# matinraayai/ir2rgb

Hardware: AMD Instinct MI355X
Metric: generator+discriminator frames/sec at 512x1024 (higher is better)
Workload: dtype bf16; 1 GPU; vid2vid training window 512x1024: 2-scale generator (composite ngf128 @256x512 + composite-local ngf64 @512x1024, tG=3) + FlowNet2 reference flow + image D (num_D=2) + 2 temporal D, 3 backward passes + Adam; batch 1 frame per GPU; parallelism=dp1 (frame-parallel sequences, RCCL gradient all-reduce)

## Files before the change

ir2rgb_amd/csrc/conv1x7_thin.hip:

```cpp
#include <utility>

#include "common.h"
#include "conv1x7_thin.h"

template <int DT, int CIN>
__global__ void __launch_bounds__(256, 1)
conv1x7_thin_kernel(const uint16_t *__restrict__ X, const uint16_t *__restrict__ Wp, float *__restrict__ Y, const T7Geom g) {
    typedef Half<DT> Hf;
    typedef typename Hf::frag frag;
    constexpr int TW = 128, KW = 7, PAD = 3, ROWS = TW + KW - 1;
    constexpr int NC = CIN / 32;
    constexpr int RB = CIN * 2;
    constexpr int RPI = 1024 / RB;
    constexpr int NDMA = (ROWS + RPI - 1) / RPI;
    constexpr int NDW = (NDMA + 3) / 4;
    constexpr int SEG = NDMA * 1024;
    __shared__ __attribute__((aligned(1024))) unsigned char smem[2 * SEG];

    const int tid = threadIdx.x, lane = tid & 63;
    const int wave = __builtin_amdgcn_readfirstlane(tid >> 6);
    const int l15 = lane & 15, grp = lane >> 4;
    const rsrc_t rx = make_rsrc(X, g.x_bytes);
    const rsrc_t rw = make_rsrc(Wp, g.w_bytes);

    frag A[KW * NC][2];
#pragma unroll
    for (int j = 0; j < KW * NC; ++j) {
        const int kx = j / NC, c = j % NC;
#pragma unroll
        for (int mt = 0; mt < 2; ++mt) {
            const int row = mt * 16 + l15;
            const unsigned off = (unsigned)((((row * (CIN / 64) + (c >> 1)) * KW + kx) * 64 + (c & 1) * 32 + grp * 8) * 2);
            typedef __attribute__((ext_vector_type(4))) unsigned u32x4;
            const u32x4 v = __builtin_amdgcn_raw_buffer_load_b128(rw, row < g.Cout ? off : IR2RGB_OOB, 0, 0);
            A[j][mt] = __builtin_bit_cast(frag, v);
        }
    }

    auto seg_coords = [&](long seg, int &n, int &y, int &x0) {
        const int sx = (int)(seg % g.nsx);
        const long r = seg / g.nsx;
        y = (int)(r % g.H);
        n = (int)(r / g.H);
        x0 = sx * TW;
    };
    auto issue = [&](long seg, int buf) {
        int n, y, x0;
        seg_coords(seg, n, y, x0);
        const unsigned rowbase = (unsigned)(((long)n * g.H + y) * g.W);
#pragma unroll
        for (int q = 0; q < NDW; ++q) {
            const int i = wave + 4 * q;
            const int row = i * RPI + (CIN == 128 ? (lane >> 4) : (lane >> 3));
            const int pos = CIN == 128 ? (lane & 15) : (lane & 7);
            const int chunk = CIN == 128 ? (pos ^ (row & 15)) : (pos ^ ((row >> 1) & 7));
            int xs = x0 - PAD + row;
            xs = xs < 0 ? -xs : xs;
            xs = xs >= g.W ? 2 * g.W - 2 - xs : xs;
            const bool ok = row < ROWS && xs >= 0 && xs < g.W && seg < g.nseg;
            const unsigned v = ok ? ((rowbase + (unsigned)xs) * (unsigned)g.ldx + (unsigned)g.ci_off + (unsigned)chunk * 8u) * 2u : IR2RGB_OOB;
            if (4 * q + 3 < NDMA || i < NDMA)
                lds_dma16(rx, v, 0, smem + buf * SEG + i * 1024);
        }
    };

    const unsigned lds0 = (unsigned)(uintptr_t)(__attribute__((address_space(3))) const unsigned char *)smem;
    unsigned base[KW];
#pragma unroll
    for (int kx = 0; kx < KW; ++kx) {
        const int row = wave * 32 + l15 + kx;
        const int f = CIN == 128 ? (row & 15) : ((row >> 1) & 7);
        base[kx] = lds0 + (unsigned)(row * RB + ((grp ^ f) & (CIN == 128 ? 15 : 7)) * 16);
    }
    constexpr int R = 8, NT = KW * NC * 2;
    auto rd = [&]<int IMM>(frag &dst, unsigned addr, std::integral_constant<int, IMM>) {
        asm volatile("ds_read_b128 %0, %1 offset:%2" : "=v"(dst) : "v"(addr), "n"(IMM) : "memory");
    };

    long seg = blockIdx.x;
    int buf = 0;
    issue(seg, 0);
    for (; seg < g.nseg; seg += gridDim.x) {
        asm volatile("s_waitcnt vmcnt(0) lgkmcnt(0)" ::: "memory");
        __builtin_amdgcn_s_barrier();
        issue(seg + gridDim.x, buf ^ 1);
        const unsigned boff = (unsigned)(buf * SEG);
        f32x4 acc[2][2];
#pragma unroll
        for (int b = 0; b < 2; ++b)
#pragma unroll
            for (int mt = 0; mt < 2; ++mt) acc[b][mt] = (f32x4){0.f, 0.f, 0.f, 0.f};
        frag B[R];
        auto fetch = [&]<int T>(std::integral_constant<int, T>) {
            constexpr int j = T / 2, bb = T % 2, kx = j / NC, c = j % NC;
            rd(B[T % R], (base[kx] ^ (unsigned)(c << 6)) + boff, std::integral_constant<int, bb * 16 * RB>{});
        };
        [&]<int... Ts>(std::integer_sequence<int, Ts...>) { (fetch(std::integral_constant<int, Ts>{}), ...); }(std::make_integer_sequence<int, R>{});
        auto body = [&]<int T>(std::integral_constant<int, T>) {
            constexpr int j = T / 2, bb = T % 2;
            constexpr int after = (NT - 1 - T) < (R - 1) ? (NT - 1 - T) : (R - 1);
            asm volatile("s_waitcnt lgkmcnt(%1)" : "+v"(B[T % R]) : "n"(after) : "memory");
            __builtin_amdgcn_sched_barrier(0);
            acc[bb][0] = Hf::mfma(A[j][0], B[T % R], acc[bb][0]);
            acc[bb][1] = Hf::mfma(A[j][1], B[T % R], acc[bb][1]);
            __builtin_amdgcn_sched_barrier(0);
            if constexpr (T + R < NT) fetch(std::integral_constant<int, T + R>{});
        };
        [&]<int... Ts>(std::integer_sequence<int, Ts...>) { (body(std::integral_constant<int, Ts>{}), ...); }(std::make_integer_sequence<int, NT>{});
        int n, y, x0;
        seg_coords(seg, n, y, x0);
#pragma unroll
        for (int b = 0; b < 2; ++b) {
            const int x = x0 + wave * 32 + b * 16 + l15;
            if (x < g.W) {
                float *dst = Y + (((long)n * g.H + y) * g.W + x) * g.ldy + g.co_off;
#pragma unroll
                for (int mt = 0; mt < 2; ++mt) {
                    const int r0 = mt * 16 + grp * 4;
                    if (r0 + 3 < g.Cout) {
                        *reinterpret_cast<float4 *>(dst + r0) = make_float4(acc[b][mt][0], acc[b][mt][1], acc[b][mt][2], acc[b][mt][3]);
                    } else {
#pragma unroll
                        for (int r = 0; r < 4; ++r)
                            if (r0 + r < g.Cout) dst[r0 + r] = acc[b][mt][r];
                    }
                }
            }
        }
        buf ^= 1;
    }
    asm volatile("s_waitcnt vmcnt(0)" ::: "memory");
}

bool conv1x7_thin_plan(const ir2rgb_conv_desc *d, const ConvView &v, T7Geom *g) {
    if (d->transposed || d->kh != 1 || d->kw != 7 || d->stride_h != 1 || d->stride_w != 1) return false;
    if (d->pad_h != 0 || d->pad_w != 3 || d->pad_mode != 1 || !d->out_f32 || d->act != 0 || d->stats_per_sample) return false;
    if (d->Cout < 1 || d->Cout > 32 || (d->Cin != 64 && d->Cin != 128) || d->Win < 4 || d->Hout != d->Hin || d->Wout != d->Win) return false;
    if (!v.half || (v.ldx & 7) || (d->ci_off & 7) || (v.ldy & 3) || (d->co_off & 3) || v.x_bytes >= (1L << 31)) return false;
    *g = T7Geom{};
    g->N = d->N; g->H = d->Hin; g->W = d->Win; g->Cout = d->Cout;
    g->ldx = v.ldx; g->ci_off = d->ci_off; g->ldy = v.ldy; g->co_off = d->co_off;
    g->nsx = (d->Win + 127) / 128;
    g->nseg = (long)d->N * d->Hin * g->nsx;
    g->x_bytes = (unsigned)v.x_bytes; g->w_bytes = (unsigned)((long)d->Cout * d->Cin * 7 * 2);
    return true;
}

int conv1x7_thin_launch(const T7Geom &g, int dtype, int cin, const void *x, const void *wp, void *y, hipStream_t s) {
    const long want = g.nseg < 512 ? g.nseg : 512;
    const unsigned grid = (unsigned)(want < 1 ? 1 : want);
    with_dtype(dtype, [&](auto dt) {
        auto launch = [&](auto kernel) { kernel<<<grid, 256, 0, s>>>((const uint16_t *)x, (const uint16_t *)wp, (float *)y, g); };
        if (cin == 128) launch(conv1x7_thin_kernel<dt.value, 128>);
        else launch(conv1x7_thin_kernel<dt.value, 64>);
    });
    return ir2rgb_launch_status();
}
```

ir2rgb_amd/csrc/conv_mfma.hip:

```cpp
#include <cstring>
#include <type_traits>
#include <utility>

#include "common.h"
#include "conv1x7_thin.h"
#include "conv3x3_patch.h"
#include "conv7x1_col.h"

#define IR2RGB_MAX_TAPS 49

struct ConvGeom {
    int N, Hin, Win, Cin;
    int Hsub, Wsub;
    int Hout, Wout, Cout;
    int s_in_y, s_in_x;
    int s_out_y, s_out_x, off_y, off_x;
    int ntaps, pad_mode;
    int kchunks;
    int act;
    int ldx, ci_off, ldy, co_off;
    int stats_row0;
    int out_f32;
    FastDiv div_hw, div_w;
    unsigned x_bytes, w_bytes;
    int cout_major;
    int ntx, dy0, dys, dx0, dxs;
    int tpi;
};


template <int TP> struct ConvTile {
    static constexpr int TC = 128;
    static constexpr int STAGE = (TC + TP) * 128;
    static constexpr int NSTAGE = TP == 128 ? 2 : 3;
    static constexpr int LDS = NSTAGE * STAGE;
};

template <int DT, int TP, int NTY, int NTX, int MROWS = 128>
__device__ __forceinline__ void
conv_igemm_body(const uint16_t *__restrict__ X, const uint16_t *__restrict__ Wp, const float *__restrict__ bias,
                uint16_t *__restrict__ Y, float *__restrict__ stats_partial, const ConvGeom &g, const int block,
                unsigned char *const smem) {
    constexpr int TC = 128;
    static_assert(MROWS == 128 || MROWS == 64 || MROWS == 32, "tile rows");
    constexpr int CW = MROWS == 64 ? 32 : 64;
    constexpr int MI = MROWS == 128 ? 4 : 2;
    constexpr int NI = TP / 64;
    constexpr int OC = MROWS <= 64 ? 64 : TC;
    constexpr int WROWS = OC / 64;
    constexpr int PROWS = TP / 64;
    constexpr int LOADS = WROWS + PROWS;
    constexpr int STAGE = (TC + TP) * 128;
    constexpr int NSTAGE = TP == 128 ? 2 : 3;
    constexpr int AHEAD = NSTAGE - 1;
    constexpr bool STATIC_TAPS = NTY > 0;
    constexpr int NT = STATIC_TAPS ? NTY * NTX : 1;
    typedef Half<DT> H;
    typedef typename H::frag frag;

    static_assert(NSTAGE * STAGE == ConvTile<TP>::LDS, "LDS ring size");

    const int tid = threadIdx.x, lane = tid & 63;
    const int wave = __builtin_amdgcn_readfirstlane(tid >> 6);
    const unsigned P = (unsigned)g.N * g.Hsub * g.Wsub;
    const unsigned HW = (unsigned)g.Hsub * g.Wsub;
    const int npt = g.tpi ? g.N * g.tpi : (int)((P + TP - 1) / TP), nct = (g.Cout + TC - 1) / TC;

    int tile;
    {
        const int nwg = npt * nct, b = block, xcd = b & 7, q = nwg >> 3, r = nwg & 7;
        if (b >= nwg) return;
        tile = (xcd < r ? xcd * (q + 1) : r * (q + 1) + (xcd - r) * q) + (b >> 3);
    }
    int pt, ct;
    if (g.cout_major) { ct = tile / npt; pt = tile - ct * npt; }
    else              { pt = tile / nct; ct = tile - pt * nct; }
    unsigned p0 = (unsigned)pt * TP, plim = P, pimg = 0;
    if (g.tpi) { pimg = (unsigned)(pt / g.tpi); p0 = (unsigned)(pt - (int)pimg * g.tpi) * TP; plim = HW; }
    auto pix_decode = [&](unsigned p, unsigned &n, unsigned &rem) {
        if (g.tpi) { n = pimg; rem = p; }
        else { n = fdiv(p, g.div_hw); rem = p - n * HW; }
    };

    const int r8 = tid >> 3, slot = tid & 7;
    const int chunk = slot ^ ((r8 >> 1) & 7);
    const long Ktot = (long)g.kchunks * g.ntaps * 64;

    const rsrc_t rw = make_rsrc(Wp, g.w_bytes), rx = make_rsrc(X, g.x_bytes);
    unsigned woff[WROWS];
#pragma unroll
    for (int i = 0; i < WROWS; ++i) {
        int co = ct * TC + r8 + 64 * i;
        co = co < g.Cout ? co : g.Cout - 1;
        woff[i] = (unsigned)(((long)co * Ktot + chunk * 8) * 2);
    }
    int psy[PROWS], psx[PROWS];
    unsigned pbase[PROWS];
#pragma unroll
    for (int i = 0; i < PROWS; ++i) {
        unsigned p = p0 + r8 + 64 * i;
        const bool v = p < plim;
        p = v ? p : 0u;
        unsigned n, rem;
        pix_decode(p, n, rem);
        unsigned sy = fdiv(rem, g.div_w);
        psy[i] = v ? (int)sy * g.s_in_y : (g.pad_mode ? 0 : -(1 << 20));
        psx[i] = (int)(rem - sy * g.Wsub) * g.s_in_x;
        pbase[i] = n * (unsigned)(g.Hin * g.Win);
    }
    unsigned char *const wave_dst = smem + wave * 1024;

    auto gather_off = [&](int i, int dy, int dx) -> unsigned {
        int iy = psy[i] + dy, ix = psx[i] + dx;
        const bool inb = ((unsigned)iy < (unsigned)g.Hin) & ((unsigned)ix < (unsigned)g.Win);
        iy = g.pad_mode ? reflect(iy, g.Hin) : iy;
        ix = g.pad_mode ? reflect(ix, g.Win) : ix;
        const unsigned off = ((pbase[i] + (unsigned)(iy * g.Win + ix)) * (unsigned)g.ldx + g.ci_off + chunk * 8) * 2u;
        return (g.pad_mode || inb) ? off : IR2RGB_OOB;
    };

    unsigned poff[STATIC_TAPS ? PROWS : 1][NT];
    if constexpr (STATIC_TAPS) {
#pragma unroll
        for (int i = 0; i < PROWS; ++i) {
            int ry[NTY > 0 ? NTY : 1], rx[NTX > 0 ? NTX : 1];
#pragma unroll
            for (int ty = 0; ty < NTY; ++ty) {
                int iy = psy[i] + g.dy0 + ty * g.dys;
                const bool in = (unsigned)iy < (unsigned)g.Hin;
                iy = g.pad_mode ? reflect(iy, g.Hin) : iy;
                ry[ty] = (g.pad_mode || in) ? iy * g.Win : -1;
            }
#pragma unroll
            for (int tx = 0; tx < NTX; ++tx) {
                int ix = psx[i] + g.dx0 + tx * g.dxs;
                const bool in = (unsigned)ix < (unsigned)g.Win;
                ix = g.pad_mode ? reflect(ix, g.Win) : ix;
                rx[tx] = (g.pad_mode || in) ? ix : -1;
            }
            const unsigned cbytes = (unsigned)(g.ci_off + chunk * 8) * 2u, ld2 = (unsigned)g.ldx * 2u;
#pragma unroll
            for (int ty = 0; ty < NTY; ++ty)
#pragma unroll
                for (int tx = 0; tx < NTX; ++tx)
                    poff[i][ty * NTX + tx] = ((ry[ty] | rx[tx]) < 0) ? IR2RGB_OOB
                                                                      : (pbase[i] + (unsigned)(ry[ty] + rx[tx])) * ld2 + cbytes;
        }
    }

    int i_cc = 0, i_ty = 0, i_tx = 0, i_t = 0;
    auto issue_weights = [&](int ks, unsigned char *dst) {
#pragma unroll
        for (int i = 0; i < WROWS; ++i) lds_dma16(rw, woff[i], (unsigned)ks * 128u, dst + 8192 * i);
    };
    auto issue_dynamic = [&](int ks, int buf) {
        unsigned char *dst = wave_dst + buf * STAGE;
        issue_weights(ks, dst);
// ... 407 lines not shown
    int Cout, Cin, T, kind;
    int bx, by;
    int entry, pad_;
};
static inline size_t pack_blocks_offset(int nentries) { return ((size_t)nentries * sizeof(PackEntry) + 15) & ~(size_t)15; }

template <int DT>
__global__ void __launch_bounds__(256)
pack_batch_kernel(const PackEntry *__restrict__ E, const PackBlock *__restrict__ B) {
    __shared__ uint16_t tile[PACK_TILE_HALFS];
    const PackBlock b = B[blockIdx.x];
    if (b.kind == 0) {
        const PackEntry &e = E[b.entry];
        pack_weight_body<DT>(b.w, b.wp, e.g, e.total, b.bx * 256L + threadIdx.x, b.by * 256L);
    } else if (b.kind == 1) {
        pack_tile_body<DT, 0>(b.w, b.wp, b.Cout, b.Cin, b.T, b.bx, b.by, tile);
    } else {
        pack_tile_body<DT, 1>(b.w, b.wp, b.Cout, b.Cin, b.T, b.bx, b.by, tile);
    }
}

struct ClassPlan {
    ConvGeom geom;
    PackGeom pack;
    long w_offset;
    int npt;
    int tp;
};

static int tile_pixels(long P, int Cout, int ksteps) {
    const long nct = (Cout + 127) / 128;
    const long tiles256 = ((P + 255) / 256) * nct;
    if (tiles256 >= 256 && ksteps >= 40) return 256;
    if (((P + 127) / 128) * nct >= 256) return 128;
    return 64;
}

static int make_plan(const ir2rgb_conv_desc *d, const ConvView &v, ClassPlan plans[4]) {
    if (!d || d->N < 1 || d->Cin < 64 || (d->Cin % 64) || d->Cout < 1 || d->kh < 1 || d->kw < 1 ||
        d->kh * d->kw > IR2RGB_MAX_TAPS || d->stride_h < 1 || d->stride_w < 1 || d->pad_h < 0 || d->pad_w < 0)
        return IR2RGB_EINVAL;
    if (!v.half) return IR2RGB_ENOSUP;
    if (d->pad_mode != 0 && d->pad_mode != 1) return IR2RGB_ENOSUP;
    int ncls = 0;
    long woff = 0;
    int row0 = 0;
    auto new_class = [&](int Hsub, int Wsub) -> ClassPlan & {
        ClassPlan &c = plans[ncls++];
        ConvGeom &g = c.geom;
        g = ConvGeom{};
        g.N = d->N; g.Hin = d->Hin; g.Win = d->Win; g.Cin = d->Cin;
        g.Hsub = Hsub; g.Wsub = Wsub; g.Hout = d->Hout; g.Wout = d->Wout; g.Cout = d->Cout;
        g.pad_mode = d->pad_mode; g.kchunks = d->Cin / 64; g.act = d->act; g.out_f32 = d->out_f32;
        c.pack = PackGeom{};
        c.pack.Cout = d->Cout; c.pack.Cin = d->Cin; c.pack.kh = d->kh; c.pack.kw = d->kw; c.pack.transposed = d->transposed ? 1 : 0;
        c.w_offset = woff;
        return c;
    };
    if (!d->transposed) {
        int Ho = (d->Hin + 2 * d->pad_h - d->kh) / d->stride_h + 1, Wo = (d->Win + 2 * d->pad_w - d->kw) / d->stride_w + 1;
        if (Ho != d->Hout || Wo != d->Wout || Ho < 1 || Wo < 1) return IR2RGB_EINVAL;
        if (d->pad_mode == 1 && (d->pad_h >= d->Hin || d->pad_w >= d->Win)) return IR2RGB_EINVAL;
        ClassPlan &c = new_class(Ho, Wo);
        ConvGeom &g = c.geom;
        g.s_in_y = d->stride_h; g.s_in_x = d->stride_w; g.s_out_y = g.s_out_x = 1; g.off_y = g.off_x = 0;
        g.ntaps = c.pack.ntaps = d->kh * d->kw;
        g.ntx = d->kw; g.dy0 = -d->pad_h; g.dys = 1; g.dx0 = -d->pad_w; g.dxs = 1;
        for (int ky = 0, t = 0; ky < d->kh; ++ky)
            for (int kx = 0; kx < d->kw; ++kx, ++t) {
                c.pack.ky[t] = (signed char)ky; c.pack.kx[t] = (signed char)kx;
            }
    } else {
        const int sh = d->stride_h, sw = d->stride_w;
        if (sh > 2 || sw > 2 || d->pad_mode != 0) return IR2RGB_ENOSUP;
        int Hfull = (d->Hin - 1) * sh - 2 * d->pad_h + d->kh, Wfull = (d->Win - 1) * sw - 2 * d->pad_w + d->kw;
        if (d->Hout < Hfull || d->Hout > Hfull + sh - 1 || d->Wout < Wfull || d->Wout > Wfull + sw - 1 || d->Hout < 1 ||
            d->Wout < 1)
            return IR2RGB_EINVAL;
        for (int a = 0; a < sh; ++a)
            for (int b = 0; b < sw; ++b) {
                const int Hsub = (d->Hout - a + sh - 1) / sh, Wsub = (d->Wout - b + sw - 1) / sw;
                if (Hsub < 1 || Wsub < 1) continue;
                ClassPlan &c = new_class(Hsub, Wsub);
                ConvGeom &g = c.geom;
                g.s_in_y = g.s_in_x = 1; g.s_out_y = sh; g.s_out_x = sw; g.off_y = a; g.off_x = b;
                int t = 0, ntx = 0;
                const int ky0 = (a + d->pad_h) % sh, kx0 = (b + d->pad_w) % sw;
                for (int ky = ky0; ky < d->kh; ky += sh) {
                    ntx = 0;
                    for (int kx = kx0; kx < d->kw; kx += sw, ++t, ++ntx) {
                        c.pack.ky[t] = (signed char)ky; c.pack.kx[t] = (signed char)kx;
                    }
                }
                if (t == 0) return IR2RGB_ENOSUP;
                g.ntx = ntx; g.dy0 = (a + d->pad_h - ky0) / sh; g.dys = -1; g.dx0 = (b + d->pad_w - kx0) / sw; g.dxs = -1;
                g.ntaps = c.pack.ntaps = t;
                woff += (long)d->Cout * d->Cin * t;
            }
    }
    if ((long)d->N * d->Hin * d->Win >= (1L << 31) || (long)d->N * d->Hout * d->Wout >= (1L << 31) ||
        (long)d->N * d->Hin * d->Win * (v.ldx / 8) >= 0xFFFFFFFFL)
        return IR2RGB_EINVAL;
    for (int i = 0; i < ncls; ++i) {
        ConvGeom &g = plans[i].geom;
        g.div_hw = make_fastdiv((unsigned)(g.Hsub * g.Wsub)); g.div_w = make_fastdiv((unsigned)g.Wsub);
        g.ldx = v.ldx; g.ci_off = d->ci_off;
        g.ldy = v.ldy; g.co_off = d->co_off;
        if (g.ci_off < 0 || g.co_off < 0 || g.ci_off + d->Cin > g.ldx || g.co_off + d->Cout > g.ldy || (g.ldx & 7) || (g.ci_off & 7))
            return IR2RGB_EINVAL;
        if ((d->Cout & 3) == 0 && ((g.ldy & 3) || (g.co_off & 3))) return IR2RGB_EINVAL;
        const long wb = (long)g.Cout * g.Cin * g.ntaps * 2;
        if (v.x_bytes >= (1L << 31) || wb >= (1L << 31)) return IR2RGB_EINVAL;
        g.x_bytes = (unsigned)v.x_bytes; g.w_bytes = (unsigned)wb;
        g.cout_major = wb > (long)g.N * g.Hin * g.Win * g.Cin * 2 ? 1 : 0;
    }
    int tp_all = 0;
    if (ncls > 1) {
        long p_all = 0, ks_sum = 0;
        for (int i = 0; i < ncls; ++i) {
            const ConvGeom &g = plans[i].geom;
            p_all += (long)g.N * g.Hsub * g.Wsub;
            ks_sum += (long)g.kchunks * g.ntaps;
        }
        tp_all = tile_pixels(p_all, plans[0].geom.Cout, (int)(ks_sum / ncls));
        const long wg128 = ((p_all + 127) / 128) * ((plans[0].geom.Cout + 127) / 128);
        if (tp_all == 128 && wg128 <= 320) tp_all = 64;
    }
    for (int i = 0; i < ncls; ++i) {
        ConvGeom &g = plans[i].geom;
        long P = (long)g.N * g.Hsub * g.Wsub;
        int tp = tp_all ? tp_all : tile_pixels(P, g.Cout, g.kchunks * g.ntaps);
        plans[i].tp = tp;
        plans[i].npt = (int)((P + tp - 1) / tp);
        if (d->stats_per_sample) {
            if (ncls > 1) return IR2RGB_ENOSUP;
            g.tpi = (int)(((long)g.Hsub * g.Wsub + tp - 1) / tp);
            plans[i].npt = g.N * g.tpi;
        }
        g.stats_row0 = row0;
        row0 += plans[i].npt;
    }
    return ncls;
}

extern "C" long ir2rgb_conv2d_packed_weight_elems(const ir2rgb_conv_desc *d) {
    ClassPlan plans[4];
    int n = make_plan(d, conv_view(d), plans);
    if (n < 0) return n;
    long e = 0;
    for (int i = 0; i < n; ++i) e += (long)d->Cout * d->Cin * plans[i].geom.ntaps;
    return e;
}

enum ConvKernel { CONV_IGEMM, CONV_CLASSES, CONV_DOT, CONV_PATCH, CONV_THIN7, CONV_COL7 };
static const char *const CONV_KERNEL_NAMES[] = {"conv_igemm_kernel", "conv_igemm_classes_kernel", "conv_dot_kernel",
                                                "conv3x3_patch_kernel", "conv1x7_thin_kernel", "conv7x1_col_kernel"};
struct ConvRoute {
    ConvKernel kernel;
    int variant;
    P3Geom p3;
    T7Geom t7;
    C7Geom c7;
    int ncls;
    ClassPlan cls[4];
    int stats_rows;
    long workspace_bytes;
};

static bool conv_dot_ok(const ir2rgb_conv_desc *d) {
    static const int v = env_switch("IR2RGB_CONV_DOT", 1);
    return v != 0 && d->out_f32 && d->Cout == 1 && !d->transposed && d->pad_mode == 0 && d->Cin >= 512 && (d->Cin % 512) == 0 &&
           d->kh * d->kw <= 16 && (d->ldx % 8) == 0 && (d->ci_off % 8) == 0;
}

static int conv_route(const ir2rgb_conv_desc *d, bool has_bias, bool has_stats, bool has_workspace, ConvRoute *r) {
    if (!d) return IR2RGB_EINVAL;
    const ConvView v = conv_view(d);
    r->stats_rows = 0; r->workspace_bytes = 0; r->ncls = 0;
    if ((r->variant = conv3x3p_plan(d, v, &r->p3, &r->stats_rows, has_workspace)) != 0) {
        r->kernel = CONV_PATCH;
        r->workspace_bytes = conv3x3p_workspace_bytes(r->variant, r->p3);
        return IR2RGB_OK;
    }
    if (conv7x1_col_plan(d, v, &r->c7)) {
        r->kernel = CONV_COL7;
        r->stats_rows = conv7x1_col_tiles(r->c7);
        return IR2RGB_OK;
    }
    if (!has_bias && !has_stats && conv1x7_thin_plan(d, v, &r->t7)) {
        r->kernel = CONV_THIN7;
        return IR2RGB_OK;
    }
    r->ncls = make_plan(d, v, r->cls);
    if (r->ncls < 0) return r->ncls;
    for (int i = 0; i < r->ncls; ++i) r->stats_rows += r->cls[i].npt;
    r->kernel = r->ncls > 1 ? CONV_CLASSES : !has_stats && conv_dot_ok(d) ? CONV_DOT : CONV_IGEMM;
    return IR2RGB_OK;
}

extern "C" const char *ir2rgb_conv2d_kernel_name(const ir2rgb_conv_desc *d) {
    ConvRoute r;
    return conv_route(d, false, false, false, &r) < 0 ? "" : CONV_KERNEL_NAMES[r.kernel];
}

extern "C" int ir2rgb_conv2d_stats_rows(const ir2rgb_conv_desc *d) {
    ConvRoute r;
    const int rc = conv_route(d, false, true, false, &r);
    return rc < 0 ? rc : r.stats_rows;
}

extern "C" long ir2rgb_conv2d_fwd_workspace_bytes(const ir2rgb_conv_desc *d) {
    ConvRoute r;
    return !d ? IR2RGB_EINVAL : conv_route(d, false, false, true, &r) < 0 ? 0 : r.workspace_bytes;
}

struct PackPlan {
    bool tiled;
    int srcCout, srcCin, T, gx, gy;
    int n;
    PackGeom g[4];
    long w_offset[4], total[4];
};

static int pack_plan(const ir2rgb_conv_desc *d, const void *w, const void *wpacked, bool adjoint, PackPlan *p) {
    ClassPlan plans[4];
    const int n = make_plan(d, conv_view(d), plans);
    if (n < 0) return n;
    if (adjoint && d->transposed) return IR2RGB_ENOSUP;
    const PackGeom &pg = plans[0].pack;
    p->T = d->kh * d->kw;
    bool natural = n == 1 && !d->transposed && pg.ntaps == p->T && p->T <= PACK_MAX_T;
    for (int t = 0; natural && t < p->T; ++t) natural = pg.ky[t] == t / d->kw && pg.kx[t] == t % d->kw;
    p->srcCout = adjoint ? d->Cin : d->Cout; p->srcCin = adjoint ? d->Cout : d->Cin;
    p->tiled = natural && p->srcCin % 64 == 0 && (!adjoint || p->srcCout % 64 == 0) && (((uintptr_t)w | (uintptr_t)wpacked) & 15) == 0;
    const int tco = adjoint ? 64 : 16, tci = adjoint ? 16 : 64;
    p->gx = p->srcCin / tci; p->gy = (p->srcCout + tco - 1) / tco;
    p->n = n;
    for (int i = 0; i < n; ++i) {
        p->g[i] = plans[i].pack;
        if (adjoint) { p->g[i].transposed = 1; p->g[i].flip = 1; }
        p->w_offset[i] = plans[i].w_offset;
        p->total[i] = (long)d->Cout * d->Cin * plans[i].geom.ntaps;
    }
    return IR2RGB_OK;
}

static int pack_impl(const ir2rgb_conv_desc *d, const float *w, void *wpacked, void *stream, bool adjoint) {
    PackPlan p;
    const int rc = pack_plan(d, w, wpacked, adjoint, &p);
    if (rc < 0) return rc;
    uint16_t *dst = reinterpret_cast<uint16_t *>(wpacked);
    hipStream_t s = as_stream(stream);
    with_dtype(d->dtype, [&](auto dt) {
        if (p.tiled) {
            auto tile = [&](auto kernel) { kernel<<<dim3((unsigned)p.gx, (unsigned)p.gy), 256, 0, s>>>(w, dst, p.srcCout, p.srcCin, p.T); };
            if (adjoint) tile(pack_tile_kernel<dt.value, 1>);
            else tile(pack_tile_kernel<dt.value, 0>);
        } else {
            for (int i = 0; i < p.n; ++i)
                pack_weight_kernel<dt.value><<<stream_grid(p.total[i], 256), 256, 0, s>>>(w, dst + p.w_offset[i], p.g[i], p.total[i]);
        }
    });
    return ir2rgb_launch_status();
}

extern "C" int ir2rgb_conv2d_pack_weight(const ir2rgb_conv_desc *d, const float *w, void *wpacked, void *stream) {
    return pack_impl(d, w, wpacked, stream, false);
}

extern "C" int ir2rgb_conv2d_pack_weight_adjoint(const ir2rgb_conv_desc *d, const float *w, void *wpacked, void *stream) {
    return pack_impl(d, w, wpacked, stream, true);
}

static int pack_entries(const ir2rgb_conv_desc *d, const float *w, void *wpacked, bool adjoint, PackEntry *out) {
    PackPlan p;
    const int rc = pack_plan(d, w, wpacked, adjoint, &p);
    if (rc < 0) return rc;
    if (!w || !wpacked) return IR2RGB_EINVAL;
    const int n = p.tiled ? 1 : p.n;
    for (int i = 0; i < n; ++i) {
        PackEntry &e = out[i];
        memset(&e, 0, sizeof(e));
        e.w = w;
        if (p.tiled) {
            e.wp = reinterpret_cast<uint16_t *>(wpacked);
            e.kind = adjoint ? 2 : 1;
            e.Cout = p.srcCout; e.Cin = p.srcCin; e.T = p.T;
            e.gx = p.gx;
            e.nblocks = p.gx * p.gy;
        } else {
            e.g = p.g[i];
            e.total = p.total[i];
            e.wp = reinterpret_cast<uint16_t *>(wpacked) + p.w_offset[i];
            const long nb = (e.total + 1023) / 1024;
            e.nblocks = (int)(nb < 1 ? 1 : (nb > 2048 ? 2048 : nb));
        }
    }
    return n;
}

static int pack_batch_expand(const ir2rgb_pack_job *jobs, int njobs, PackEntry *E, int max_entries, long *nblocks) {
    if (!jobs || njobs < 1) return IR2RGB_EINVAL;
    int n = 0;
    long blocks = 0;
    for (int j = 0; j < njobs; ++j) {
        if (jobs[j].desc.dtype != jobs[0].desc.dtype) return IR2RGB_EINVAL;
        PackEntry tmp[4];
        const int k = pack_entries(&jobs[j].desc, (const float *)jobs[j].w, jobs[j].wpacked, jobs[j].adjoint != 0, tmp);
        if (k < 0) return k;
        for (int i = 0; i < k; ++i) {
            tmp[i].first_block = (int)blocks;
            blocks += tmp[i].nblocks;
            if (E) {
                if (n >= max_entries) return IR2RGB_EINVAL;
                E[n] = tmp[i];
            }
            ++n;
        }
    }
    if (blocks > 0x7fffffffL) return IR2RGB_EINVAL;
    *nblocks = blocks;
    return n;
}

extern "C" long ir2rgb_conv2d_pack_batch_table_bytes(const ir2rgb_pack_job *jobs, int njobs) {
    long blocks = 0;
    const int n = pack_batch_expand(jobs, njobs, nullptr, 0, &blocks);
    if (n < 0) return n;
    return (long)(pack_blocks_offset(n) + (size_t)blocks * sizeof(PackBlock));
}

extern "C" int ir2rgb_conv2d_pack_batch_build(const ir2rgb_pack_job *jobs, int njobs, void *table_host, long table_bytes,
                                              int *nblocks) {
    if (!table_host || !nblocks) return IR2RGB_EINVAL;
    const long need = ir2rgb_conv2d_pack_batch_table_bytes(jobs, njobs);
    if (need < 0) return (int)need;
    if (table_bytes < need) return IR2RGB_EINVAL;
    PackEntry *E = reinterpret_cast<PackEntry *>(table_host);
    long blocks = 0;
    const int n = pack_batch_expand(jobs, njobs, E, (int)(table_bytes / (long)sizeof(PackEntry)), &blocks);
    if (n < 0) return n;
    PackBlock *B = reinterpret_cast<PackBlock *>(reinterpret_cast<char *>(table_host) + pack_blocks_offset(n));
    for (int i = 0; i < n; ++i) {
        const PackEntry &e = E[i];
        for (int lb = 0; lb < e.nblocks; ++lb) {
            PackBlock &b = B[e.first_block + lb];
            memset(&b, 0, sizeof(b));
            b.w = e.w; b.wp = e.wp; b.Cout = e.Cout; b.Cin = e.Cin; b.T = e.T; b.kind = e.kind; b.entry = i;
            if (e.kind == 0) { b.bx = lb; b.by = e.nblocks; }
            else { b.bx = lb % e.gx; b.by = lb / e.gx; }
        }
    }
    *nblocks = (int)blocks;
    return n;
}

extern "C" int ir2rgb_conv2d_pack_batch_run(const void *table_dev, int nentries, int nblocks, int dtype, void *stream) {
    if (!table_dev || nentries < 1 || nblocks < 1) return IR2RGB_EINVAL;
    if (dtype != IR2RGB_BF16 && dtype != IR2RGB_F16) return IR2RGB_ENOSUP;
    if ((uintptr_t)table_dev & 15) return IR2RGB_EALIGN;
    const PackEntry *E = reinterpret_cast<const PackEntry *>(table_dev);
    const PackBlock *B = reinterpret_cast<const PackBlock *>(reinterpret_cast<const char *>(table_dev) + pack_blocks_offset(nentries));
    with_dtype(dtype, [&](auto dt) { pack_batch_kernel<dt.value><<<nblocks, 256, 0, as_stream(stream)>>>(E, B); });
    return ir2rgb_launch_status();
}

template <class F> static void with_tile(int tp, F &&f) {
    switch (tp) {
        case 256: f(std::integral_constant<int, 256>{}); break;
        case 128: f(std::integral_constant<int, 128>{}); break;
        default:  f(std::integral_constant<int, 64>{}); break;
    }
}

template <int NTY, int NTX> struct Taps {};

static int tile_rows(int Cout, bool thin_ok) {
    static const int half = env_switch("IR2RGB_CONV_HALF_TILE", 1);
    return Cout <= 32 && thin_ok ? 32 : Cout <= 64 && half != 0 ? 64 : 128;
}

static void launch_conv(const ClassPlan &c, int dtype, const uint16_t *x, const uint16_t *wp, const float *bias, uint16_t *y,
                        float *stats, hipStream_t s) {
    const ConvGeom &g = c.geom;
    const unsigned grid = (unsigned)(c.npt * ((g.Cout + 127) / 128));
    const int nty = g.ntaps / g.ntx;
    const int mrows = tile_rows(g.Cout, (nty == 4 && g.ntx == 4) || (nty == 1 && g.ntx == 7));
    auto launch = [&]<int NTY, int NTX>(Taps<NTY, NTX>) {
        with_dtype(dtype, [&](auto dt) {
            with_tile(c.tp, [&](auto tp) {
                auto go = [&](auto mr) {
                    conv_igemm_kernel<dt.value, tp.value, NTY, NTX, mr.value><<<grid, 512, 0, s>>>(x, wp, bias, y, stats, g);
                };
                if constexpr ((NTY == 4 && NTX == 4) || (NTY == 1 && NTX == 7)) {
                    if (mrows == 32) return go(std::integral_constant<int, 32>{});
                }
                if (mrows == 64) go(std::integral_constant<int, 64>{});
                else             go(std::integral_constant<int, 128>{});
            });
        });
    };
    if (nty == 3 && g.ntx == 3)      launch(Taps<3, 3>{});
    else if (nty == 4 && g.ntx == 4) launch(Taps<4, 4>{});
    else if (nty == 7 && g.ntx == 1) launch(Taps<7, 1>{});
    else if (nty == 1 && g.ntx == 7) launch(Taps<1, 7>{});
    else if (nty == 4 && g.ntx == 1) launch(Taps<4, 1>{});
    else if (nty == 2 && g.ntx == 2) launch(Taps<2, 2>{});
    else if (nty == 2 && g.ntx == 1) launch(Taps<2, 1>{});
    else if (nty == 1 && g.ntx == 2) launch(Taps<1, 2>{});
    else if (nty == 1 && g.ntx == 1) launch(Taps<1, 1>{});
    else                             launch(Taps<0, 0>{});
}

static void launch_classes(const ClassPlan *plans, int n, int dtype, const uint16_t *x, const uint16_t *wp, const float *bias,
                           uint16_t *y, float *stats, hipStream_t s) {
    ConvClasses cs;
    int order[4] = {0, 1, 2, 3};
    for (int i = 0; i < n; ++i)
        for (int j = i + 1; j < n; ++j)
            if (plans[order[j]].geom.ntaps > plans[order[i]].geom.ntaps) { int t = order[i]; order[i] = order[j]; order[j] = t; }
    int first = 0;
    for (int i = 0; i < n; ++i) {
        const ClassPlan &c = plans[order[i]];
        cs.g[i] = c.geom;
        cs.w_off[i] = c.w_offset;
        cs.first[i] = first;
        const int nwg = c.npt * ((c.geom.Cout + 127) / 128);
        first += (nwg + 7) & ~7;
    }
    cs.first[n] = first;
    cs.n = n;
    with_dtype(dtype, [&](auto dt) {
        with_tile(plans[0].tp, [&](auto tp) {
            if (tile_rows(plans[0].geom.Cout, false) == 64)
                conv_igemm_classes_kernel<dt.value, tp.value, 64><<<first, 512, 0, s>>>(x, wp, bias, y, stats, cs);
            else
                conv_igemm_classes_kernel<dt.value, tp.value, 128><<<first, 512, 0, s>>>(x, wp, bias, y, stats, cs);
        });
    });
}

extern "C" int ir2rgb_conv2d_fwd_ws(const ir2rgb_conv_desc *d, const void *x, const void *wpacked, const float *bias,
                                    void *y, float *stats_partial, void *workspace, long workspace_bytes, void *stream) {
    if (!d) return IR2RGB_EINVAL;
    if ((((uintptr_t)x | (uintptr_t)wpacked | (uintptr_t)y) & 15) != 0) return IR2RGB_EALIGN;
    ConvRoute r;
    const int rc = conv_route(d, bias != nullptr, stats_partial != nullptr, workspace != nullptr, &r);
    if (rc < 0) return rc;
    hipStream_t s = as_stream(stream);
    const uint16_t *X = (const uint16_t *)x, *W = (const uint16_t *)wpacked;
    switch (r.kernel) {
        case CONV_PATCH: return conv3x3p_launch(r.variant, r.p3, d->dtype, x, wpacked, bias, y, stats_partial, s, workspace, workspace_bytes);
        case CONV_COL7: return conv7x1_col_launch(r.c7, d->dtype, x, wpacked, bias, y, stats_partial, s);
        case CONV_THIN7: return conv1x7_thin_launch(r.t7, d->dtype, d->Cin, x, wpacked, y, s);
        case CONV_DOT: {
            const ConvGeom &g = r.cls[0].geom;
            const long P = (long)g.N * g.Hout * g.Wout;
            const long waves = P < 8192 ? P : 8192;
            with_dtype(d->dtype, [&](auto dt) { conv_dot_kernel<dt.value><<<(unsigned)((waves + 3) / 4), 256, 0, s>>>(X, W, bias, (float *)y, g); });
            break;
        }
        case CONV_CLASSES: launch_classes(r.cls, r.ncls, d->dtype, X, W, bias, (uint16_t *)y, stats_partial, s); break;
        case CONV_IGEMM: launch_conv(r.cls[0], d->dtype, X, W, bias, (uint16_t *)y, stats_partial, s); break;
    }
    return ir2rgb_launch_status();
}

extern "C" int ir2rgb_conv2d_fwd(const ir2rgb_conv_desc *d, const void *x, const void *wpacked, const float *bias,
                                 void *y, float *stats_partial, void *stream) {
    return ir2rgb_conv2d_fwd_ws(d, x, wpacked, bias, y, stats_partial, nullptr, 0, stream);
}
```

Baseline: 40.66 frames/s.

## Add dedicated row-tiled MFMA kernel for 1x7 zero-pad convs with Cin 64

Adds a new conv1x7 row kernel for 1x7 convolutions with zero padding, Cin 64 and Cout 64 or 128. It keeps the weights in registers, double-buffers 128-pixel row segments into LDS via DMA, and writes bf16 output with bias through buffer stores. The router picks it ahead of the generic implicit-GEMM path when no stats are needed, aiming to cut overhead on these layers. It also switches segment index math in the thin kernel to 32-bit unsigned to reduce scalar division cost. The new path is on by default and can be disabled with an environment switch.

```diff
diff --git a/ir2rgb_amd/csrc/conv1x7_row.h b/ir2rgb_amd/csrc/conv1x7_row.h
--- /dev/null
+++ b/ir2rgb_amd/csrc/conv1x7_row.h
@@ -0,0 +1,13 @@
+#pragma once
+#include "common.h"
+
+struct R7Geom {
+    int N, H, Win, Wout, Cout;
+    int pad;
+    int ldx, ci_off, ldy, co_off;
+    int nsx;
+    long nseg;
+    unsigned x_bytes, y_bytes, w_bytes;
+};
+bool conv1x7_row_plan(const ir2rgb_conv_desc *d, const ConvView &v, R7Geom *g);
+int conv1x7_row_launch(const R7Geom &g, int dtype, const void *x, const void *wp, const float *bias, void *y, hipStream_t s);
diff --git a/ir2rgb_amd/csrc/conv1x7_row.hip b/ir2rgb_amd/csrc/conv1x7_row.hip
--- /dev/null
+++ b/ir2rgb_amd/csrc/conv1x7_row.hip
@@ -0,0 +1,165 @@
+#include <utility>
+
+#include "common.h"
+#include "conv1x7_row.h"
+
+template <int DT, int COUT>
+__global__ void __launch_bounds__(256, COUT == 64 ? 2 : 1)
+conv_igemm_row7_kernel(const uint16_t *__restrict__ X, const uint16_t *__restrict__ Wp, const float *__restrict__ bias,
+                       uint16_t *__restrict__ Y, const R7Geom g) {
+    typedef Half<DT> Hf;
+    typedef typename Hf::frag frag;
+    constexpr int TW = 128, KW = 7, ROWS = TW + KW - 1;
+    constexpr int RB = 128, RPI = 8;
+    constexpr int NDMA = (ROWS + RPI - 1) / RPI, NDW = (NDMA + 3) / 4;
+    constexpr int SEG = NDMA * 1024;
+    constexpr int WC = COUT / 32, WP = 4 / WC;
+    constexpr int NB = TW / 16 / WP;
+    constexpr int NKS = KW * 2;
+    __shared__ __attribute__((aligned(1024))) unsigned char smem[2 * SEG];
+
+    const int tid = threadIdx.x, lane = tid & 63;
+    const int wave = __builtin_amdgcn_readfirstlane(tid >> 6);
+    const int wc = wave % WC, wp = wave / WC;
+    const int l15 = lane & 15, grp = lane >> 4;
+    const rsrc_t rx = make_rsrc(X, g.x_bytes);
+    const rsrc_t rw = make_rsrc(Wp, g.w_bytes);
+    const rsrc_t ry = make_rsrc(Y, g.y_bytes);
+
+    frag A[NKS][2];
+#pragma unroll
+    for (int j = 0; j < NKS; ++j) {
+        const int kx = j >> 1, c = j & 1;
+#pragma unroll
+        for (int mt = 0; mt < 2; ++mt) {
+            const int co = wc * 32 + (l15 >> 2) * 8 + mt * 4 + (l15 & 3);
+            const unsigned off = (unsigned)(((co * KW + kx) * 64 + c * 32 + grp * 8) * 2);
+            A[j][mt] = __builtin_bit_cast(frag, __builtin_amdgcn_raw_buffer_load_b128(rw, off, 0, 0));
+        }
+    }
+    const int co0 = wc * 32 + grp * 8;
+    float bv[2][4];
+#pragma unroll
+    for (int mt = 0; mt < 2; ++mt)
+#pragma unroll
+        for (int r = 0; r < 4; ++r) bv[mt][r] = bias != nullptr ? bias[co0 + mt * 4 + r] : 0.f;
+
+    const unsigned nseg = (unsigned)g.nseg;
+    auto seg_coords = [&](unsigned seg, int &n, int &y, int &x0) {
+        const unsigned r = seg / (unsigned)g.nsx;
+        x0 = (int)(seg - r * (unsigned)g.nsx) * TW;
+        n = (int)(r / (unsigned)g.H);
+        y = (int)(r - (unsigned)n * (unsigned)g.H);
+    };
+    auto issue = [&](unsigned seg, int buf) {
+        int n, y, x0;
+        seg_coords(seg, n, y, x0);
+        const unsigned rowbase = (unsigned)(((long)n * g.H + y) * g.Win);
+#pragma unroll
+        for (int q = 0; q < NDW; ++q) {
+            const int i = wave + 4 * q;
+            const int row = i * RPI + (lane >> 3), pos = lane & 7, chunk = pos ^ ((row >> 1) & 7);
+            const int xs = x0 - g.pad + row;
+            const bool ok = row < ROWS && xs >= 0 && xs < g.Win && seg < nseg;
+            const unsigned v = ok ? ((rowbase + (unsigned)xs) * (unsigned)g.ldx + (unsigned)g.ci_off + (unsigned)chunk * 8u) * 2u : IR2RGB_OOB;
+            if (4 * q + 3 < NDMA || i < NDMA)
+                lds_dma16(rx, v, 0, smem + buf * SEG + i * 1024);
+        }
+    };
+
+    const unsigned lds0 = (unsigned)(uintptr_t)(__attribute__((address_space(3))) const unsigned char *)smem;
+    unsigned base[KW];
+#pragma unroll
+    for (int kx = 0; kx < KW; ++kx) {
+        const int row = wp * NB * 16 + l15 + kx;
+        base[kx] = lds0 + (unsigned)(row * RB + ((grp ^ (row >> 1)) & 7) * 16);
+    }
+    static_assert(((WP - 1) * NB * 16 + 15 + KW - 1 + (NB - 1) * 16 + 1) * RB <= SEG, "reads stay inside the segment");
+    constexpr int R = 8, NT = NKS * NB;
+    auto rd = [&]<int IMM>(frag &dst, unsigned addr, std::integral_constant<int, IMM>) {
+        asm volatile("ds_read_b128 %0, %1 offset:%2" : "=v"(dst) : "v"(addr), "n"(IMM) : "memory");
+    };
+
+    unsigned seg = blockIdx.x;
+    int buf = 0;
+    issue(seg, 0);
+    for (; seg < nseg; seg += gridDim.x) {
+        asm volatile("s_waitcnt vmcnt(0) lgkmcnt(0)" ::: "memory");
+        __builtin_amdgcn_s_barrier();
+        issue(seg + gridDim.x, buf ^ 1);
+        const unsigned boff = (unsigned)(buf * SEG);
+        f32x4 acc[NB][2];
+#pragma unroll
+        for (int b = 0; b < NB; ++b)
+#pragma unroll
+            for (int mt = 0; mt < 2; ++mt) acc[b][mt] = (f32x4){0.f, 0.f, 0.f, 0.f};
+        frag B[R];
+        auto fetch = [&]<int T>(std::integral_constant<int, T>) {
+            constexpr int j = T / NB, bb = T % NB, kx = j >> 1, c = j & 1;
+            rd(B[T % R], (base[kx] ^ (unsigned)(c << 6)) + boff, std::integral_constant<int, bb * 16 * RB>{});
+        };
+        [&]<int... Ts>(std::integer_sequence<int, Ts...>) { (fetch(std::integral_constant<int, Ts>{}), ...); }(std::make_integer_sequence<int, R>{});
+        auto body = [&]<int T>(std::integral_constant<int, T>) {
+            constexpr int j = T / NB, bb = T % NB;
+            constexpr int after = (NT - 1 - T) < (R - 1) ? (NT - 1 - T) : (R - 1);
+            asm volatile("s_waitcnt lgkmcnt(%1)" : "+v"(B[T % R]) : "n"(after) : "memory");
+            __builtin_amdgcn_sched_barrier(0);
+            acc[bb][0] = Hf::mfma(A[j][0], B[T % R], acc[bb][0]);
+            acc[bb][1] = Hf::mfma(A[j][1], B[T % R], acc[bb][1]);
+            __builtin_amdgcn_sched_barrier(0);
+            if constexpr (T + R < NT) fetch(std::integral_constant<int, T + R>{});
+        };
+        [&]<int... Ts>(std::integer_sequence<int, Ts...>) { (body(std::integral_constant<int, Ts>{}), ...); }(std::make_integer_sequence<int, NT>{});
+        int n, y, x0;
+        seg_coords(seg, n, y, x0);
+        const unsigned outrow = (unsigned)(((long)n * g.H + y) * g.Wout);
+#pragma unroll
+        for (int b = 0; b < NB; ++b) {
+            const int x = x0 + (wp * NB + b) * 16 + l15;
+            typedef __attribute__((ext_vector_type(4))) unsigned u32x4;
+            u32x4 pk;
+            pk.x = (uint32_t)Hf::cvt(acc[b][0][0] + bv[0][0]) | ((uint32_t)Hf::cvt(acc[b][0][1] + bv[0][1]) << 16);
+            pk.y = (uint32_t)Hf::cvt(acc[b][0][2] + bv[0][2]) | ((uint32_t)Hf::cvt(acc[b][0][3] + bv[0][3]) << 16);
+            pk.z = (uint32_t)Hf::cvt(acc[b][1][0] + bv[1][0]) | ((uint32_t)Hf::cvt(acc[b][1][1] + bv[1][1]) << 16);
+            pk.w = (uint32_t)Hf::cvt(acc[b][1][2] + bv[1][2]) | ((uint32_t)Hf::cvt(acc[b][1][3] + bv[1][3]) << 16);
+            const unsigned off = ((outrow + (unsigned)x) * (unsigned)g.ldy + (unsigned)(g.co_off + co0)) * 2u;
+            __builtin_amdgcn_raw_buffer_store_b128(pk, ry, x < g.Wout ? off : IR2RGB_OOB, 0, 0);
+        }
+        buf ^= 1;
+    }
+    asm volatile("s_waitcnt vmcnt(0)" ::: "memory");
+}
+
+static bool row7_enabled() {
+    static const int v = env_switch("IR2RGB_CONV7_ROW", 1);
+    return v != 0;
+}
+
+bool conv1x7_row_plan(const ir2rgb_conv_desc *d, const ConvView &v, R7Geom *g) {
+    if (!row7_enabled() || d->transposed || d->kh != 1 || d->kw != 7 || d->stride_h != 1 || d->stride_w != 1) return false;
+    if (d->pad_h != 0 || d->pad_w < 0 || d->pad_w > 6 || d->pad_mode != 0 || d->out_f32 || d->act != 0 || d->stats_per_sample) return false;
+    if (d->Cin != 64 || (d->Cout != 64 && d->Cout != 128) || d->N < 1 || d->Hin < 1 || d->Win < 7) return false;
+    if (d->Hout != d->Hin || d->Wout != d->Win + 2 * d->pad_w - 6) return false;
+    if (!v.half || (v.ldx & 7) || (d->ci_off & 7) || (v.ldy & 7) || (d->co_off & 7)) return false;
+    if (d->ci_off < 0 || d->co_off < 0 || d->ci_off + 64 > v.ldx || d->co_off + d->Cout > v.ldy) return false;
+    if (v.x_bytes >= (1L << 31) || v.y_bytes >= (1L << 31)) return false;
+    const int nsx = (d->Wout + 127) / 128;
+    const long nseg = (long)d->N * d->Hin * nsx;
+    if ((double)(nsx * 128) / d->Wout > 1.13 || nseg < 200) return false;
+    *g = R7Geom{};
+    g->N = d->N; g->H = d->Hin; g->Win = d->Win; g->Wout = d->Wout; g->Cout = d->Cout; g->pad = d->pad_w;
+    g->ldx = v.ldx; g->ci_off = d->ci_off; g->ldy = v.ldy; g->co_off = d->co_off;
+    g->nsx = nsx; g->nseg = nseg;
+    g->x_bytes = (unsigned)v.x_bytes; g->y_bytes = (unsigned)v.y_bytes; g->w_bytes = (unsigned)((long)d->Cout * 64 * 7 * 2);
+    return true;
+}
+
+int conv1x7_row_launch(const R7Geom &g, int dtype, const void *x, const void *wp, const float *bias, void *y, hipStream_t s) {
+    const unsigned grid = (unsigned)(g.nseg < 512 ? g.nseg : 512);
+    with_dtype(dtype, [&](auto dt) {
+        auto launch = [&](auto kernel) { kernel<<<grid, 256, 0, s>>>((const uint16_t *)x, (const uint16_t *)wp, bias, (uint16_t *)y, g); };
+        if (g.Cout == 128) launch(conv_igemm_row7_kernel<dt.value, 128>);
+        else launch(conv_igemm_row7_kernel<dt.value, 64>);
+    });
+    return ir2rgb_launch_status();
+}
diff --git a/ir2rgb_amd/csrc/conv1x7_thin.hip b/ir2rgb_amd/csrc/conv1x7_thin.hip
--- a/ir2rgb_amd/csrc/conv1x7_thin.hip
+++ b/ir2rgb_amd/csrc/conv1x7_thin.hip
@@ -37,14 +37,14 @@
         }
     }
 
-    auto seg_coords = [&](long seg, int &n, int &y, int &x0) {
-        const int sx = (int)(seg % g.nsx);
-        const long r = seg / g.nsx;
-        y = (int)(r % g.H);
-        n = (int)(r / g.H);
-        x0 = sx * TW;
+    const unsigned nseg = (unsigned)g.nseg;
+    auto seg_coords = [&](unsigned seg, int &n, int &y, int &x0) {
+        const unsigned r = seg / (unsigned)g.nsx;
+        x0 = (int)(seg - r * (unsigned)g.nsx) * TW;
+        n = (int)(r / (unsigned)g.H);
+        y = (int)(r - (unsigned)n * (unsigned)g.H);
     };
-    auto issue = [&](long seg, int buf) {
+    auto issue = [&](unsigned seg, int buf) {
         int n, y, x0;
         seg_coords(seg, n, y, x0);
         const unsigned rowbase = (unsigned)(((long)n * g.H + y) * g.W);
@@ -57,7 +57,7 @@
             int xs = x0 - PAD + row;
             xs = xs < 0 ? -xs : xs;
             xs = xs >= g.W ? 2 * g.W - 2 - xs : xs;
-            const bool ok = row < ROWS && xs >= 0 && xs < g.W && seg < g.nseg;
+            const bool ok = row < ROWS && xs >= 0 && xs < g.W && seg < nseg;
             const unsigned v = ok ? ((rowbase + (unsigned)xs) * (unsigned)g.ldx + (unsigned)g.ci_off + (unsigned)chunk * 8u) * 2u : IR2RGB_OOB;
             if (4 * q + 3 < NDMA || i < NDMA)
                 lds_dma16(rx, v, 0, smem + buf * SEG + i * 1024);
@@ -77,10 +77,10 @@
         asm volatile("ds_read_b128 %0, %1 offset:%2" : "=v"(dst) : "v"(addr), "n"(IMM) : "memory");
     };
 
-    long seg = blockIdx.x;
+    unsigned seg = blockIdx.x;
     int buf = 0;
     issue(seg, 0);
-    for (; seg < g.nseg; seg += gridDim.x) {
+    for (; seg < nseg; seg += gridDim.x) {
         asm volatile("s_waitcnt vmcnt(0) lgkmcnt(0)" ::: "memory");
         __builtin_amdgcn_s_barrier();
         issue(seg + gridDim.x, buf ^ 1);
diff --git a/ir2rgb_amd/csrc/conv_mfma.hip b/ir2rgb_amd/csrc/conv_mfma.hip
--- a/ir2rgb_amd/csrc/conv_mfma.hip
+++ b/ir2rgb_amd/csrc/conv_mfma.hip
@@ -3,6 +3,7 @@
 #include <utility>
 
 #include "common.h"
+#include "conv1x7_row.h"
 #include "conv1x7_thin.h"
 #include "conv3x3_patch.h"
 #include "conv7x1_col.h"
@@ -716,15 +717,17 @@
     return e;
 }
 
-enum ConvKernel { CONV_IGEMM, CONV_CLASSES, CONV_DOT, CONV_PATCH, CONV_THIN7, CONV_COL7 };
+enum ConvKernel { CONV_IGEMM, CONV_CLASSES, CONV_DOT, CONV_PATCH, CONV_THIN7, CONV_COL7, CONV_ROW7 };
 static const char *const CONV_KERNEL_NAMES[] = {"conv_igemm_kernel", "conv_igemm_classes_kernel", "conv_dot_kernel",
-                                                "conv3x3_patch_kernel", "conv1x7_thin_kernel", "conv7x1_col_kernel"};
+                                                "conv3x3_patch_kernel", "conv1x7_thin_kernel", "conv7x1_col_kernel",
+                                                "conv_igemm_kernel"};
 struct ConvRoute {
     ConvKernel kernel;
     int variant;
     P3Geom p3;
     T7Geom t7;
     C7Geom c7;
+    R7Geom r7;
     int ncls;
     ClassPlan cls[4];
     int stats_rows;
@@ -758,6 +761,10 @@
     r->ncls = make_plan(d, v, r->cls);
     if (r->ncls < 0) return r->ncls;
     for (int i = 0; i < r->ncls; ++i) r->stats_rows += r->cls[i].npt;
+    if (!has_stats && conv1x7_row_plan(d, v, &r->r7)) {
+        r->kernel = CONV_ROW7;
+        return IR2RGB_OK;
+    }
     r->kernel = r->ncls > 1 ? CONV_CLASSES : !has_stats && conv_dot_ok(d) ? CONV_DOT : CONV_IGEMM;
     return IR2RGB_OK;
 }
@@ -1017,6 +1024,7 @@
         case CONV_PATCH: return conv3x3p_launch(r.variant, r.p3, d->dtype, x, wpacked, bias, y, stats_partial, s, workspace, workspace_bytes);
         case CONV_COL7: return conv7x1_col_launch(r.c7, d->dtype, x, wpacked, bias, y, stats_partial, s);
         case CONV_THIN7: return conv1x7_thin_launch(r.t7, d->dtype, d->Cin, x, wpacked, y, s);
+        case CONV_ROW7: return conv1x7_row_launch(r.r7, d->dtype, x, wpacked, bias, y, s);
         case CONV_DOT: {
             const ConvGeom &g = r.cls[0].geom;
             const long P = (long)g.N * g.Hout * g.Wout;
```

New measurement: 38.99 frames/s. -4.1%, worse.
